# indiejoseph/speech-distill

Measured on AMD Instinct MI355X. Metric: distill-step tokens/sec (student seq_len=512), higher is better.
Workload: dtype bf16; 1 GPU; BASELINE config 2: Qwen3-0.6B-shape student + SoulX-1.7B-shape teacher (random init), V=159488, batch 4/GPU, seq_len 512, top_k 128, T=2.0 alpha=0.5, student fwd+bwd + teacher fwd + top-K + KL/CE; global_batch=4, seq_len=512, parallelism=single

## Files before the change

### include/sd_hip.h

```cpp
#pragma once
#include <stdint.h>
#ifdef __cplusplus
extern "C" {
#endif

#define SD_OK 0
#define SD_ERR_SHAPE (-1)
#define SD_ERR_ALIGN (-2)
#define SD_ERR_UNSUPPORTED (-3)
#define SD_ERR_NO_TEACHER (-4)
#define SD_ERR_WORKSPACE (-5)

#define SD_DTYPE_BF16 0
#define SD_DTYPE_F32 1

int sd_abi_version(void);

int sd_gemm_bf16(const void* A, const void* B, void* C, const void* R, int M, int N, int K, int64_t lda,
                 int64_t ldb, int64_t ldc, int64_t ldr, int trans_a, int trans_b, void* stream);

int sd_gemm_splitk_plan(int M, int N, int K);
int64_t sd_gemm_splitk_workspace_bytes(int M, int N, int K);
int sd_gemm_bf16_splitk(const void* A, const void* B, void* C, const void* R, int M, int N, int K, int64_t lda,
                        int64_t ldb, int64_t ldc, int64_t ldr, int trans_a, int trans_b, void* workspace,
// ... 60 lines not shown
int sd_qknorm_rope_bwd(const void* dqk, const void* qkv, const void* q_gain, const void* k_gain, const void* cos_tab,
                       const void* sin_tab, void* dqkv, void* dq_gain, void* dk_gain, int accumulate_dw, void* workspace,
                       int M, int T, int Hq, int Hkv, float eps, void* stream);

int sd_swiglu_fwd(const void* gate_up, void* act, int M, int I, void* stream);
int sd_swiglu_bwd(const void* dact, const void* gate_up, void* dgate_up, int M, int I, void* stream);

int sd_embedding_fwd(const int64_t* ids, const void* E, void* x, int M, int H, int V, void* stream);
int sd_embedding_bwd(const int64_t* ids, const void* dx, void* dE, int M, int H, int V, float scale, void* stream);
int sd_rows_scatter(const void* src, const int64_t* rows, void* dst, int n, int M, int H, void* stream);

int sd_attn_fwd(const void* q, const void* k, const void* v, void* o, float* lse, const int32_t* kv_len, int64_t ldq,
                int64_t ldk, int64_t ldv, int64_t ldo, int B, int T, int Hq, int Hkv, int head_dim, float scale,
                void* stream);
int sd_attn_bwd(const void* q, const void* k, const void* v, const void* o, const void* d_o, const float* lse,
                float* delta, void* dq, void* dk, void* dv, const int32_t* kv_len, int64_t ldq, int64_t ldk, int64_t ldv,
                int64_t ldo, int64_t lddq, int64_t lddk, int64_t lddv, int B, int T, int Hq, int Hkv, int head_dim,
                float scale, void* stream);

int sd_attn_bwd2(const void* q, const void* k, const void* v, const void* o, const void* d_o, const float* lse,
                 float* delta, void* dq, void* dk, void* dv, const int32_t* kv_len, int64_t ldq, int64_t ldk, int64_t ldv,
                 int64_t ldo, int64_t lddq, int64_t lddk, int64_t lddv, int B, int T, int Hq, int Hkv, int head_dim,
                 float scale, void* side_stream, void* stream);

int sd_logsoftmax_topk(const void* logits, void* top_v, void* top_i, float* lse_out, int rows, int64_t row_stride,
                       int V, int K, int dtype, void* stream);

int sd_loss_rows(const int64_t* labels, const int64_t* speech_mask, const int64_t* mask_a, const int64_t* mask_b,
                 int64_t* rows, int64_t* row_labels, int32_t* meta, int B, int T, void* stream);

int64_t sd_kdloss_stats_bytes(int B, int T);
int sd_kdloss_fwd(const void* student_logits, const void* teacher_logits, const void* top_k_v, const void* top_k_i,
                  const int64_t* labels, const uint8_t* speech_mask, void* row_stats, float* loss_out, int B, int T, int V,
                  int K, float temperature, float alpha, int dtype, void* stream);
int sd_kdloss_bwd(const void* student_logits, const void* teacher_logits, const void* top_k_v, const void* top_k_i,
                  const int64_t* labels, const void* row_stats, const float* loss_out, const float* grad_total,
                  void* grad_logits, int B, int T, int V, int K, float temperature, float alpha, int dtype, void* stream);

int sd_kdloss_fwd_rows(const void* student_logits, const void* teacher_logits, const void* top_k_v, const void* top_k_i,
                       const int64_t* row_labels, void* row_stats, float* loss_out, int R, int V, int K,
                       float temperature, float alpha, int dtype, void* stream);
int sd_kdloss_bwd_rows(const void* student_logits, const void* teacher_logits, const void* top_k_v, const void* top_k_i,
                       const int64_t* row_labels, const void* row_stats, const float* loss_out, const float* grad_total,
                       void* grad_logits, int R, int V, int K, float temperature, float alpha, int dtype, void* stream);

#define SD_SUMSQ_PARTIALS 2048
// ... 86 lines not shown
```

### speech_distill_amd/_lib.py

```python
from __future__ import annotations

import ctypes as C
import os

_HERE = os.path.dirname(os.path.abspath(__file__))
_LIB = None

ERRORS = {-1: "SD_ERR_SHAPE", -2: "SD_ERR_ALIGN", -3: "SD_ERR_UNSUPPORTED", -4: "SD_ERR_NO_TEACHER",
          -5: "SD_ERR_WORKSPACE"}


class SdHipError(RuntimeError):
    pass


def lib_path() -> str:
    return os.environ.get("SD_HIP_LIB") or os.path.join(_HERE, "libsd_hip.so")


class Dims(C.Structure):
    _fields_ = [("vocab", C.c_int32), ("hidden", C.c_int32), ("inter", C.c_int32), ("layers", C.c_int32),
                ("n_q", C.c_int32), ("n_kv", C.c_int32), ("head_dim", C.c_int32), ("tied", C.c_int32),
                ("eps", C.c_float), ("pad_", C.c_int32)]

# ... 52 lines not shown
    "sd_rmsnorm_bwd_workspace_bytes": (_i64, [_i, _i]),
    "sd_rmsnorm_bwd": (_i, [_vp, _vp, _vp, _vp, _vp, _vp, _vp, _i, _vp, _i, _i, _vp]),
    "sd_gemm_swiglu": (_i, [_vp, _vp, _vp, _vp, _i, _i, _i, _vp]),
    "sd_gemm_qkv_rope": (_i, [_vp, _vp, _vp, _vp, _vp, _vp, _vp, _vp, _i, _i, _i, _i, _i, _f, _vp]),
    "sd_embedding_fwd_ssq": (_i, [_vp, _vp, _vp, _vp, _i, _i, _i, _vp]),
    "sd_gemm_bf16_ssq": (_i, [_vp, _vp, _vp, _vp, _vp, _i, _i, _i, _i64, _i64, _i64, _i64, _vp]),
    "sd_gemm_qkv_rope_rs": (_i, [_vp, _vp, _vp, _vp, _vp, _vp, _vp, _vp, _vp, _i, _i, _i, _i, _i, _f, _vp]),
    "sd_gemm_swiglu_rs": (_i, [_vp, _vp, _vp, _vp, _vp, _f, _i, _i, _i, _vp]),
    "sd_qwen3_fold_supported": (_i, [C.POINTER(Dims)]),
    "sd_gemm_bf16_splitk_partial": (_i, [_vp, _vp, _vp, _i, _i, _i, _i64, _i64, _i64, _i, _i, _vp, _i64, _vp, _vp]),
    "sd_rmsnorm_bwd_slabs": (_i, [_vp, _i, _vp, _vp, _vp, _vp, _vp, _vp, _i, _vp, _i, _i, _vp, _vp, _vp]),
    "sd_rmsnorm_bwd2": (_i, [_vp, _vp, _vp, _vp, _vp, _vp, _vp, _i, _vp, _i, _i, _vp, _vp, _vp]),
    "sd_qknorm_rope_bwd2": (_i, [_vp, _vp, _vp, _vp, _vp, _vp, _vp, _vp, _vp, _i, _vp, _i, _i, _i, _i, _f, _vp, _vp, _vp]),
    "sd_qknorm_rope_fwd": (_i, [_vp, _vp, _vp, _vp, _vp, _vp, _i, _i, _i, _i, _f, _vp]),
    "sd_qknorm_rope_bwd_workspace_bytes": (_i64, [_i, _i, _i]),
    "sd_qknorm_rope_bwd": (_i, [_vp, _vp, _vp, _vp, _vp, _vp, _vp, _vp, _vp, _i, _vp, _i, _i, _i, _i, _f, _vp]),
    "sd_swiglu_fwd": (_i, [_vp, _vp, _i, _i, _vp]),
    "sd_swiglu_bwd": (_i, [_vp, _vp, _vp, _i, _i, _vp]),
    "sd_embedding_fwd": (_i, [_vp, _vp, _vp, _i, _i, _i, _vp]),
    "sd_embedding_bwd": (_i, [_vp, _vp, _vp, _i, _i, _i, _f, _vp]),
    "sd_attn_fwd": (_i, [_vp, _vp, _vp, _vp, _vp, _vp, _i64, _i64, _i64, _i64, _i, _i, _i, _i, _i, _f, _vp]),
    "sd_attn_bwd": (_i, [_vp] * 11 + [_i64] * 7 + [_i, _i, _i, _i, _i, _f, _vp]),
    "sd_attn_bwd2": (_i, [_vp] * 11 + [_i64] * 7 + [_i, _i, _i, _i, _i, _f, _vp, _vp]),
    "sd_logsoftmax_topk": (_i, [_vp, _vp, _vp, _vp, _i, _i64, _i, _i, _i, _vp]),
    "sd_kdloss_stats_bytes": (_i64, [_i, _i]),
    "sd_kdloss_fwd": (_i, [_vp, _vp, _vp, _vp, _vp, _vp, _vp, _vp, _i, _i, _i, _i, _f, _f, _i, _vp]),
    "sd_kdloss_bwd": (_i, [_vp, _vp, _vp, _vp, _vp, _vp, _vp, _vp, _vp, _i, _i, _i, _i, _f, _f, _i, _vp]),
    "sd_gemm_grouped_tn": (_i, [_vp, _i, _i, _i, _vp]),
    "sd_gemm_swiglu_bwd": (_i, [_vp, _vp, _vp, _vp, _i, _i, _i, _vp]),
    "sd_gemm_odx_delta": (_i, [_vp, _vp, _vp, _vp, _i64, _vp, _i, _i, _i, _i, _vp]),
    "sd_kdloss_fwd_rows": (_i, [_vp, _vp, _vp, _vp, _vp, _vp, _vp, _i, _i, _i, _f, _f, _i, _vp]),
    "sd_kdloss_bwd_rows": (_i, [_vp, _vp, _vp, _vp, _vp, _vp, _vp, _vp, _vp, _i, _i, _i, _f, _f, _i, _vp]),
    "sd_rows_scatter": (_i, [_vp, _vp, _vp, _i, _i, _i, _vp]),
    "sd_loss_rows": (_i, [_vp, _vp, _vp, _vp, _vp, _vp, _vp, _i, _i, _vp]),
    "sd_rmsnorm_bwd_partial_rows": (_i, [_i, _i]),
    "sd_qknorm_rope_bwd_partial_rows": (_i, [_i, _i, _i]),
    "sd_colsum_reduce_batch": (_i, [_vp, _i, _vp]),
    "sd_sumsq_bf16": (_i, [_vp, _i64, _vp, _vp, _vp]),
    "sd_adamw_bf16": (_i, [_vp, _vp, _vp, _vp, _i64, _f, _f, _f, _f, _f, _i, _vp, _f, _vp]),
    "sd_lora_plan_bytes": (_i64, [_i]),
    "sd_lora_plan_build": (_i, [C.POINTER(LoraTarget), _i, _i, _vp, _i64]),
    "sd_lora_merge": (_i, [_vp, _vp, _vp]),
    "sd_lora_project": (_i, [_vp, _vp, _vp]),
    "sd_adamw_f32_shadow": (_i, [_vp, _vp, _vp, _vp, _vp, _vp, _f, _i64, _f, _f, _f, _f, _f, _i, _vp, _f, _vp]),
    "sd_streams_overlap": (_i, [_vp, _vp, _f, C.POINTER(C.c_int)]),
    "sd_prof_begin": (_i, []),
# ... 68 lines not shown
```

### speech_distill_amd/csrc/sd_attn.hip

```cpp
#include <type_traits>
#include "sd_common.cuh"
#include "../../include/sd_hip.h"
#include "sd_prof.h"
#include "sd_debug.h"
#include "sd_events.h"

namespace {

constexpr int D = 128;
constexpr int TILE = 64 * D * 2;
constexpr float NEG = -1.0e30f;
constexpr float LOG2E = 1.4426950408889634f;

SD_DEV int f_swz(int row) { return ((row & 3) << 2) | ((row >> 2) & 3); }

template <int NP = 4>
struct TileDma {
  int voff[NP];
  long row_bytes;
#if defined(__HIP_DEVICE_COMPILE__)
  __amdgpu_buffer_rsrc_t rsrc;
#endif
  SD_DEV void init(const bf16* g, long ld, int rows, int w, int lane) {
    row_bytes = ld * 2;
// ... 33 lines not shown
  sd_u64 raw[8];
#pragma unroll
  for (int db = 0; db < 4; ++db) {
    const int ch = db * 4 + chl;
    lds_tr16_pair_asm(raw[2 * db], raw[2 * db + 1], aA + ((ch ^ sA) << 4), aB + ((ch ^ sB) << 4));
  }
  lds_tr_wait8(raw);
#pragma unroll
  for (int db = 0; db < 4; ++db) out[db] = cat8_u64(raw[2 * db], raw[2 * db + 1]);
}

SD_DEV void tr_issue4(const char* lds, int rb, int lane, sd_u64 (&raw)[8]) {
  const int gi = lane >> 4, i = lane & 15, q4 = i >> 2, pp = i & 3;
  const int rA = rb + 4 * (gi >> 1) + q4, rB = rA + 8;
  const int sA = f_swz(rA), sB = f_swz(rB);
  const unsigned base = lds_addr(lds) + 8 * (pp & 1);
  const unsigned aA = base + rA * 256, aB = base + rB * 256;
  const int chl = (gi & 1) * 2 + (pp >> 1);
#pragma unroll
  for (int db = 0; db < 4; ++db) {
    const int ch = db * 4 + chl;
    lds_tr16_pair_asm(raw[2 * db], raw[2 * db + 1], aA + ((ch ^ sA) << 4), aB + ((ch ^ sB) << 4));
  }
}
SD_DEV void tr_finish4(sd_u64 (&raw)[8], bf16x8 (&out)[4]) {
  lds_tr_wait8(raw);
#pragma unroll
  for (int db = 0; db < 4; ++db) out[db] = cat8_u64(raw[2 * db], raw[2 * db + 1]);
}

SD_DEV float halves_max(float x) {
  float a = x, b = x;
  asm volatile("s_nop 1\n\tv_permlane32_swap_b32 %0, %1\n\ts_nop 0" : "+v"(a), "+v"(b));
  return fmaxf(a, b);
}

SD_DEV bf16x8 acc_frag(const f32x16& p, int s) {
  bf16x8 r;
#pragma unroll
  for (int j = 0; j < 8; ++j) r[j] = (bf16)p[8 * s + j];
  return r;
}

SD_DEV int acc_row(int reg, int h) { return (reg & 3) + 8 * (reg >> 2) + 4 * h; }

SD_DEV void store_tile_rows(char* img, const f32x16 (&acc)[4], float mul, bf16* g_row0, long ld, int rows_valid, int lane) {
// ... 568 lines not shown
          for (int db = 0; db < 4; ++db) acc[db] = mfma32(kt4[db], df, acc[db]);
        }
      }
    }
  }
  asm volatile("s_waitcnt vmcnt(0)" ::: "memory");
  __syncthreads();
  float* xo = (float*)smem + (long)w * 64 * 64;
  if (half == 1) {
#pragma unroll
    for (int db = 0; db < 4; ++db)
#pragma unroll
      for (int e = 0; e < 16; ++e) xo[(db * 16 + e) * 64 + lane] = acc[db][e];
  }
  __syncthreads();
  if (half == 1 || !active) return;
#pragma unroll
  for (int db = 0; db < 4; ++db)
#pragma unroll
    for (int e = 0; e < 16; ++e) acc[db][e] += xo[(db * 16 + e) * 64 + lane];
  store_tile_rows((char*)xo, acc, scale, dQ + (tok0 + q0w) * lddq + hq * D, lddq, T - q0w, lane);
}

__global__ __launch_bounds__(512) void attn_bwd_dkv_kernel(const bf16* __restrict__ Q, const bf16* __restrict__ Kp,
                                                           const bf16* __restrict__ Vp, const bf16* __restrict__ dO,
                                                           const float* __restrict__ LSE, const float* __restrict__ delta,
                                                           bf16* __restrict__ dK, bf16* __restrict__ dV,
                                                           const int* __restrict__ kv_len, long ldq, long ldk, long ldv,
                                                           long ldo, long lddk, long lddv, int T, int Hq, int Hkv,
                                                           float scale) {
  __shared__ __attribute__((aligned(16))) char smem[8 * TILE + 1024];
  const int lane = lane_id(), w8 = wave_id_uniform();
  const int grp = w8 >> 2, sub = w8 & 1, rh = (w8 >> 1) & 1;
  const int sw = w8 & 3;
  const int G = Hq / Hkv;
  const int n64 = (T + 63) / 64;
  const AttnWg wg = attn_wg((int)blockIdx.x, (n64 + 1) / 2, 1, Hkv, (int)gridDim.x / (((n64 + 1) / 2) * Hkv));
  const int hkv = wg.hkv, b = wg.b;
  const int kbA = wg.pair, kbB = n64 - 1 - wg.pair;
  const bool active = grp == 0 || kbB != kbA;
  const int k0w = (grp == 0 ? kbA : kbB) * 64 + 32 * sub;
  const int r = lane & 31, h = lane >> 5;
  const int klen = kv_len ? max(1, min(kv_len[b], T)) : T;
  const long tok0 = (long)b * T;
  const int key = k0w + r;
  const bool key_ok = key < klen;
  const float c = scale * LOG2E;
  char* const ksm = smem;
  char* const vsm = smem + 2 * TILE;
  char* const ring = smem + 4 * TILE;
  float* const stat = (float*)(smem + 8 * TILE);
  {
    TileDma<> kvd;
    kvd.init((grp ? Vp + tok0 * ldv : Kp + tok0 * ldk) + hkv * D, grp ? ldv : ldk, T, sw, lane);
// ... 46 lines not shown
    const int qb0 = (qt0 + it % per_head) * 64 + 32 * rh;
    if (!active || qb0 + 31 < k0w) continue;
    f32x16 s, dp;
#pragma unroll
    for (int e = 0; e < 16; ++e) { s[e] = 0.f; dp[e] = 0.f; }
#pragma unroll
    for (int st = 0; st < 8; ++st) {
      s = mfma32(row_frag(qs, 32 * rh, st, lane), row_frag(ksm, 64 * grp + 32 * sub, st, lane), s);
      dp = mfma32(row_frag(dos, 32 * rh, st, lane), row_frag(vsm, 64 * grp + 32 * sub, st, lane), dp);
    }
#pragma unroll
    for (int g4 = 0; g4 < 4; ++g4) {
      const f32x4 l2 = *(const f32x4*)&stat[buf * 128 + 32 * rh + 8 * g4 + 4 * h];
      const f32x4 dl = *(const f32x4*)&stat[buf * 128 + 64 + 32 * rh + 8 * g4 + 4 * h];
#pragma unroll
      for (int e = 0; e < 4; ++e) {
        const int qq = qb0 + 8 * g4 + 4 * h + e;
        const bool vis = key_ok && key <= qq && qq < T;
        const float p = vis ? __builtin_amdgcn_exp2f(s[4 * g4 + e] * c - l2[e]) : 0.f;
        s[4 * g4 + e] = p;
        dp[4 * g4 + e] = p * (dp[4 * g4 + e] - dl[e]);
      }
    }
#pragma unroll
    for (int ss = 0; ss < 2; ++ss) {
      bf16x8 t4[4];
      const bf16x8 pf = acc_frag(s, ss);
      tr_frag4(dos, 32 * rh + 16 * ss, lane, t4);
#pragma unroll
      for (int db = 0; db < 4; ++db) dv[db] = mfma32(t4[db], pf, dv[db]);
      const bf16x8 df = acc_frag(dp, ss);
      tr_frag4(qs, 32 * rh + 16 * ss, lane, t4);
#pragma unroll
      for (int db = 0; db < 4; ++db) dk[db] = mfma32(t4[db], df, dk[db]);
    }
  }
  asm volatile("s_waitcnt vmcnt(0) lgkmcnt(0)" ::: "memory");
  __syncthreads();
  float* xo = (float*)smem + (long)(grp * 2 + sub) * 64 * 64;
#pragma unroll
  for (int round = 0; round < 2; ++round) {
    f32x16* acc = round ? dv : dk;
    if (rh == 1) {
#pragma unroll
      for (int db = 0; db < 4; ++db)
#pragma unroll
        for (int e = 0; e < 16; ++e) xo[(db * 16 + e) * 64 + lane] = acc[db][e];
    }
    __syncthreads();
    if (rh == 0) {
#pragma unroll
      for (int db = 0; db < 4; ++db)
#pragma unroll
        for (int e = 0; e < 16; ++e) acc[db][e] += xo[(db * 16 + e) * 64 + lane];
    }
    __syncthreads();
  }
  if (rh == 0 && active) {
    store_tile_rows((char*)xo, dk, scale, dK + (tok0 + k0w) * lddk + hkv * D, lddk, T - k0w, lane);
    store_tile_rows((char*)xo + 8192, dv, 1.f, dV + (tok0 + k0w) * lddv + hkv * D, lddv, T - k0w, lane);
  }
}

int check_common(int B, int T, int Hq, int Hkv, long ldq, long ldk, long ldv, long ldo) {
  if (B <= 0 || T <= 0 || Hq <= 0 || Hkv <= 0 || (Hq % Hkv)) return SD_ERR_SHAPE;
  if ((ldq | ldk | ldv | ldo) & 7) return SD_ERR_ALIGN;
  return 0;
}

}

#ifdef SD_STAMPS
static unsigned long long* g_attn_stamps = nullptr;
extern "C" void sd_debug_attn_stamp_buffer(void* p) { g_attn_stamps = (unsigned long long*)p; }
#define SD_ATT_STAMP_ARG , g_attn_stamps
#else
#define SD_ATT_STAMP_ARG
#endif


extern "C" int sd_attn_fwd(const void* q, const void* k, const void* v, void* o, float* lse, const int32_t* kv_len,
                           int64_t ldq, int64_t ldk, int64_t ldv, int64_t ldo, int B, int T, int Hq, int Hkv,
                           int head_dim, float scale, void* stream) {
  if (head_dim != D) return SD_ERR_UNSUPPORTED;
  if (int e = check_common(B, T, Hq, Hkv, ldq, ldk, ldv, ldo)) return e;
  if (((uintptr_t)q | (uintptr_t)k | (uintptr_t)v | (uintptr_t)o) & 15) return SD_ERR_ALIGN;
  SdProfScope prof(SD_K_ATTN_FWD, 2.0 * B * Hq * (double)T * T * D, (hipStream_t)stream);
  const dim3 grid((((T + 63) / 64 + 1) / 2) * Hq * B);
  const bool pipe = (g_sd_debug.attn_variant & 2) || (!(g_sd_debug.attn_variant & 1) && T >= 1024);
  if (pipe) {
    hipLaunchKernelGGL(attn_fwd_pipe_kernel, grid, dim3(512), 0, (hipStream_t)stream, (const bf16*)q, (const bf16*)k,
                       (const bf16*)v, (bf16*)o, lse, kv_len, ldq, ldk, ldv, ldo, T, Hq, Hkv, scale SD_ATT_STAMP_ARG);
    SD_CHECK_LAUNCH();
    return 0;
  }
  hipLaunchKernelGGL(attn_fwd_kernel, grid, dim3(512), 0, (hipStream_t)stream, (const bf16*)q,
                     (const bf16*)k, (const bf16*)v, (bf16*)o, lse, kv_len, ldq, ldk, ldv, ldo, T, Hq, Hkv, scale SD_ATT_STAMP_ARG);
  SD_CHECK_LAUNCH();
  return 0;
}

extern "C" int sd_attn_bwd2(const void* q, const void* k, const void* v, const void* o, const void* d_o, const float* lse,
                            float* delta, void* dq, void* dk, void* dv, const int32_t* kv_len, int64_t ldq, int64_t ldk,
                            int64_t ldv, int64_t ldo, int64_t lddq, int64_t lddk, int64_t lddv, int B, int T, int Hq,
                            int Hkv, int head_dim, float scale, void* side_stream, void* stream) {
  if (head_dim != D) return SD_ERR_UNSUPPORTED;
  if (int e = check_common(B, T, Hq, Hkv, ldq, ldk, ldv, ldo)) return e;
  if ((lddq | lddk | lddv) & 7) return SD_ERR_ALIGN;
  hipStream_t st = (hipStream_t)stream, s2 = (hipStream_t)side_stream;
  SdEventLease lease;
  if (s2 && !(lease.set = sd_lease_events())) return SD_ERR_WORKSPACE;
  hipEvent_t* g_attn_ev = lease.set ? lease.set->ev : nullptr;
  const long total = (long)B * T * Hq;
  if (o) {
    hipLaunchKernelGGL(attn_delta_kernel, dim3((unsigned)((total + 15) / 16)), dim3(256), 0, st, (const bf16*)d_o,
                       (const bf16*)o, delta, ldo, T, Hq, total);
    SD_CHECK_LAUNCH();
  }
  hipStream_t sq = s2 ? s2 : st;
  if (s2) {
    if (hipEventRecord(g_attn_ev[0], st) != hipSuccess || hipStreamWaitEvent(s2, g_attn_ev[0], 0) != hipSuccess)
      return SD_ERR_WORKSPACE;
  }
  {
    SdProfScope prof2(SD_K_ATTN_BWD_DQ, 3.0 * B * Hq * (double)T * T * D, sq);
    hipLaunchKernelGGL(attn_bwd_dq_kernel, dim3((((T + 63) / 64 + 1) / 2) * Hq * B), dim3(512), 0, sq, (const bf16*)q, (const bf16*)k,
                       (const bf16*)v, (const bf16*)d_o, lse, (const float*)delta, (bf16*)dq, kv_len, ldq, ldk, ldv, ldo,
                       lddq, T, Hq, Hkv, scale);
  }
  SD_CHECK_LAUNCH();
  {
    SdProfScope prof(SD_K_ATTN_BWD_DKV, 4.0 * B * Hq * (double)T * T * D, st);
    hipLaunchKernelGGL(attn_bwd_dkv_kernel, dim3((((T + 63) / 64 + 1) / 2) * Hkv * B), dim3(512), 0, st, (const bf16*)q,
                       (const bf16*)k, (const bf16*)v, (const bf16*)d_o, lse, (const float*)delta, (bf16*)dk, (bf16*)dv,
                       kv_len, ldq, ldk, ldv, ldo, lddk, lddv, T, Hq, Hkv, scale);
  }
  SD_CHECK_LAUNCH();
  if (s2) {
    if (hipEventRecord(g_attn_ev[1], s2) != hipSuccess || hipStreamWaitEvent(st, g_attn_ev[1], 0) != hipSuccess)
      return SD_ERR_WORKSPACE;
  }
  return 0;
}

extern "C" int sd_attn_bwd(const void* q, const void* k, const void* v, const void* o, const void* d_o, const float* lse,
                           float* delta, void* dq, void* dk, void* dv, const int32_t* kv_len, int64_t ldq, int64_t ldk,
                           int64_t ldv, int64_t ldo, int64_t lddq, int64_t lddk, int64_t lddv, int B, int T, int Hq,
                           int Hkv, int head_dim, float scale, void* stream) {
  return sd_attn_bwd2(q, k, v, o, d_o, lse, delta, dq, dk, dv, kv_len, ldq, ldk, ldv, ldo, lddq, lddk, lddv, B, T, Hq,
                      Hkv, head_dim, scale, nullptr, stream);
}
```

### speech_distill_amd/csrc/sd_debug.h

```cpp
#pragma once

struct SdDebug {
  int gemm_force_bm = 0, gemm_force_nst = 0;
  int gemm_checked_staging = 0;
  int gemm_p256_unpaired = 0;
  int gemm_cu_budget = 0;
  int gemm_no_persist = 0, gemm_no_p256 = 0;
  int gemm_p256_min_tiles = 1024;
  int gemm_group_m = 0;
  int gemm_tn_stag_min = 1024;
  int gemm_splitk_min_kt = 96, gemm_splitk_min_slice = 24;
  int gemm_splitk_max = 0;
  int gemm_fwd_cu_budget = 0;
  int gemm_persist_balance = 0;
  int gemm_no_table = 0;
  int gemm_fwd_bump = 0;
  int model_fuse_student_swiglu = 0;
  int model_shared_layers = -1, model_shared_layers_train = -1;
  int model_overlap_mask = 31;
  int topk_nt = 0;
  int qk_bwd_blocks = 512;
  int attn_variant = 0;
};
extern SdDebug g_sd_debug;

extern thread_local int t_sd_shared_gpu;
struct SdSharedGpuScope {
  int prev;
  explicit SdSharedGpuScope(int on) : prev(t_sd_shared_gpu) { t_sd_shared_gpu = on; }
  ~SdSharedGpuScope() { t_sd_shared_gpu = prev; }
};
```

### speech_distill_amd/csrc/sd_debug.hip

```cpp
#include <stdint.h>
#include <string.h>
#include "../../include/sd_hip.h"
#include "../../include/sd_hip_debug.h"
#include "sd_debug.h"

SdDebug g_sd_debug;
thread_local int t_sd_shared_gpu = 0;

namespace {
struct Key { const char* name; int SdDebug::*field; };
const Key kKeys[] = {
    {"gemm.force_bm", &SdDebug::gemm_force_bm},
    {"gemm.force_nst", &SdDebug::gemm_force_nst},
    {"gemm.checked_staging", &SdDebug::gemm_checked_staging},
    {"gemm.p256_unpaired", &SdDebug::gemm_p256_unpaired},
    {"gemm.cu_budget", &SdDebug::gemm_cu_budget},
    {"gemm.no_persist", &SdDebug::gemm_no_persist},
    {"gemm.no_p256", &SdDebug::gemm_no_p256},
    {"gemm.p256_min_tiles", &SdDebug::gemm_p256_min_tiles},
    {"gemm.group_m", &SdDebug::gemm_group_m},
    {"gemm.tn_stag_min", &SdDebug::gemm_tn_stag_min},
    {"gemm.splitk_min_kt", &SdDebug::gemm_splitk_min_kt},
    {"gemm.splitk_min_slice", &SdDebug::gemm_splitk_min_slice},
    {"gemm.splitk_max", &SdDebug::gemm_splitk_max},
    {"gemm.no_table", &SdDebug::gemm_no_table},
    {"gemm.persist_balance", &SdDebug::gemm_persist_balance},
    {"gemm.fwd_cu_budget", &SdDebug::gemm_fwd_cu_budget},
    {"gemm.fwd_bump", &SdDebug::gemm_fwd_bump},
    {"model.fuse_student_swiglu", &SdDebug::model_fuse_student_swiglu},
    {"model.overlap_mask", &SdDebug::model_overlap_mask},
    {"model.shared_layers", &SdDebug::model_shared_layers},
    {"model.shared_layers_train", &SdDebug::model_shared_layers_train},
    {"topk.nt", &SdDebug::topk_nt},
    {"qk_bwd.blocks", &SdDebug::qk_bwd_blocks},
    {"attn.variant", &SdDebug::attn_variant},
};
}

extern "C" int sd_debug_set(const char* key, int64_t value) {
  if (!key) return SD_ERR_SHAPE;
  if (!strcmp(key, "reset")) { g_sd_debug = SdDebug{}; return SD_OK; }
  for (const Key& k : kKeys)
    if (!strcmp(key, k.name)) {
      if (k.field == &SdDebug::gemm_splitk_min_slice && value < 1) value = 1;
      g_sd_debug.*(k.field) = (int)value;
      return SD_OK;
    }
  return SD_ERR_UNSUPPORTED;
}

extern "C" int64_t sd_debug_get(const char* key) {
  if (key)
    for (const Key& k : kKeys)
      if (!strcmp(key, k.name)) return g_sd_debug.*(k.field);
  return INT64_MIN;
}

extern "C" int sd_debug_keys(char* buf, int cap) {
// ... 10 lines not shown
```

### speech_distill_amd/csrc/sd_model.hip

```cpp
#include <hip/hip_runtime.h>
#include <stdint.h>
#include <stdlib.h>
#include "../../include/sd_hip.h"
#include "sd_events.h"
#include "sd_debug.h"

namespace {

inline int64_t al(int64_t x) { return (x + 255) & ~(int64_t)255; }

struct Sizes {
  int M, h, I, QD, KD, QKV, QK, V, L, Hq, Hkv;
  int64_t x, rstd, qkv, qk, ao, lse, gu, act;
  Sizes(const sd_qwen3_dims* d, int B, int T) {
    M = B * T; h = d->hidden; I = d->inter; Hq = d->n_q; Hkv = d->n_kv;
    QD = Hq * d->head_dim; KD = Hkv * d->head_dim; QKV = QD + 2 * KD; QK = QD + KD; V = d->vocab; L = d->layers;
    x = al((int64_t)M * h * 2); rstd = al((int64_t)M * 4); qkv = al((int64_t)M * QKV * 2); qk = al((int64_t)M * QK * 2);
    ao = al((int64_t)M * QD * 2); lse = al((int64_t)B * Hq * T * 4); gu = al((int64_t)M * 2 * I * 2);
    act = al((int64_t)M * I * 2);
  }
  int64_t per_layer() const { return 4 * x + 2 * rstd + qkv + qk + ao + lse + gu + act; }
  int64_t tail() const { return 3 * x + rstd; }
  int64_t ssq() const { return al((int64_t)M * 16 * 4); }
  int64_t body(int save) const {
    return save == SD_SAVE_ALL ? (int64_t)L * per_layer() : save == SD_SAVE_LAYER_INPUTS ? (int64_t)L * x + 2 * per_layer()
                                                                                          : per_layer() + x;
  }
};

struct LayerActs {
  char *x_in, *rstd1, *xn1, *qkv, *qk, *ao, *lse, *x_mid, *rstd2, *xn2, *gu, *act;
};

LayerActs carve(const Sizes& s, char* p) {
  LayerActs a;
  a.x_in = p; p += s.x;
  a.rstd1 = p; p += s.rstd;
  a.xn1 = p; p += s.x;
  a.qkv = p; p += s.qkv;
  a.qk = p; p += s.qk;
  a.ao = p; p += s.ao;
  a.lse = p; p += s.lse;
  a.x_mid = p; p += s.x;
  a.rstd2 = p; p += s.rstd;
  a.xn2 = p; p += s.x;
  a.gu = p; p += s.gu;
  a.act = p; p += s.act;
  return a;
}

struct BwdScratch {
  char *dxa[2], *dxb[2], *dqkv[2], *dgu[2], *ws_norm2[2], *ws_qk[2], *ws_norm1[2];
  char *dxn, *dqk, *dao, *delta, *dact, *ws_norm, *ws_splitk;
  int64_t total, splitk_bytes;
  BwdScratch(const Sizes& s, char* p) {
    char* p0 = p;
    for (int i = 0; i < 2; ++i) {
      dxa[i] = p; p += s.x;
      dxb[i] = p; p += s.x;
      dqkv[i] = p; p += s.qkv;
      dgu[i] = p; p += s.gu;
      ws_norm2[i] = p; p += al(sd_rmsnorm_bwd_workspace_bytes(s.M, s.h));
      ws_qk[i] = p; p += al(sd_qknorm_rope_bwd_workspace_bytes(s.M, s.Hq, s.Hkv));
      ws_norm1[i] = p; p += al(sd_rmsnorm_bwd_workspace_bytes(s.M, s.h));
    }
    dxn = p; p += s.x;
    dqk = p; p += s.qk;
    dao = p; p += s.ao;
    delta = p; p += s.lse;
    dact = p; p += s.act;
    ws_norm = p; p += al(sd_rmsnorm_bwd_workspace_bytes(s.M, s.h));
    splitk_bytes = sd_gemm_splitk_workspace_bytes(s.M, s.h, s.V);
    for (int k : {s.QKV, 2 * s.I, s.QD, s.I}) {
      const int64_t b1 = sd_gemm_splitk_workspace_bytes(s.M, s.h, k);
      splitk_bytes = b1 > splitk_bytes ? b1 : splitk_bytes;
    }
    ws_splitk = p; p += al(splitk_bytes);
    total = p - p0;
  }
};

#define RUN(call) do { int e__ = (call); if (e__) return e__; } while (0)

LayerActs layer_acts(const Sizes& s, char* base, int l, int save) {
  if (save == SD_SAVE_ALL) return carve(s, base + (int64_t)l * s.per_layer());
  LayerActs a = carve(s, base + (int64_t)s.L * s.x + (int64_t)(l & 1) * s.per_layer());
  a.x_in = base + (int64_t)l * s.x;
  return a;
}

int layer_forward(const sd_qwen3_dims* d, const Sizes& s, const LayerActs& a, const sd_qwen3_layer& w, char* x_out,
                  bool keep_gu, const int32_t* kv_len, const void* cos_tab, const void* sin_tab, int B, int T,
                  void* stream) {
  const float scale = 0.08838834764831845f;
  RUN(sd_rmsnorm_fwd(a.x_in, w.ln1, a.xn1, (float*)a.rstd1, s.M, s.h, d->eps, stream));
  int rc = sd_gemm_qkv_rope(a.xn1, w.wqkv, a.qkv, a.qk, w.q_gain, w.k_gain, cos_tab, sin_tab, s.M, T, s.Hq, s.Hkv, s.h,
                            d->eps, stream);
  if (rc == SD_ERR_UNSUPPORTED) {
    RUN(sd_gemm_bf16(a.xn1, w.wqkv, a.qkv, nullptr, s.M, s.QKV, s.h, s.h, s.h, s.QKV, 0, 0, 0, stream));
    RUN(sd_qknorm_rope_fwd(a.qkv, w.q_gain, w.k_gain, cos_tab, sin_tab, a.qk, s.M, T, s.Hq, s.Hkv, d->eps, stream));
// ... 241 lines not shown
      const int rc = sd_gemm_swiglu_bwd(dx_in, w.wdown, a.gu, dgu, s.M, s.I, s.h, stream);
      if (rc == SD_ERR_UNSUPPORTED) {
        RUN(sd_gemm_bf16(dx_in, w.wdown, b.dact, nullptr, s.M, s.I, s.h, s.h, s.I, s.I, 0, 0, 1, stream));
        RUN(sd_swiglu_bwd(b.dact, a.gu, dgu, s.M, s.I, stream));
      } else if (rc) {
        return rc;
      }
    }
    if (!grouped) SIGNAL(1);
    RUN(sd_gemm_bf16_splitk_partial(dgu, w.wgu, b.dxn, s.M, s.h, 2 * s.I, 2 * s.I, s.h, s.h, 0, 1, b.ws_splitk,
                                    b.splitk_bytes, &nsp, stream));
    if (!grouped) RUN(sd_gemm_bf16(dgu, a.xn2, gw.wgu, ACC(gw.wgu), 2 * s.I, s.h, s.M, 2 * s.I, s.h, s.h, s.h, 1, 1, wstream));
    NORM_BWD(a.x_mid, w.ln2, (const float*)a.rstd2, dx_in, dxb, batch_gains ? nullptr : gw.ln2, b.ws_norm2[P],
             (ovl & 2) ? side_stream : nullptr, s2 ? (void*)g_ev[8] : nullptr);
    if (!grouped) SIGNAL(2);
    const void* o_for_delta = a.ao;
    {
      const int rc = sd_gemm_odx_delta(dxb, w.wo, b.dao, a.ao, s.QD, (float*)b.delta, s.M, T, s.Hq, s.h, stream);
      if (rc == SD_ERR_UNSUPPORTED) RUN(sd_gemm_bf16(dxb, w.wo, b.dao, nullptr, s.M, s.QD, s.h, s.h, s.QD, s.QD, 0, 0, 1, stream));
      else if (rc) return rc;
      else o_for_delta = nullptr;
    }
    if (!grouped) RUN(sd_gemm_bf16(dxb, a.ao, gw.wo, ACC(gw.wo), s.h, s.QD, s.M, s.h, s.QD, s.QD, s.QD, 1, 1, wstream));
    RUN(sd_attn_bwd2(a.qk, a.qk + (int64_t)s.QD * 2, a.qkv + (int64_t)(s.QD + s.KD) * 2, o_for_delta, b.dao, (const float*)a.lse,
                    (float*)b.delta, b.dqk, b.dqk + (int64_t)s.QD * 2, dqkv + (int64_t)(s.QD + s.KD) * 2, kv_len, s.QK,
                    s.QK, s.QKV, s.QD, s.QK, s.QK, s.QKV, B, T, s.Hq, s.Hkv, 128, scale, (ovl & 4) ? side_stream : nullptr, stream));
    RUN(sd_qknorm_rope_bwd2(b.dqk, a.qkv, w.q_gain, w.k_gain, cos_tab, sin_tab, dqkv, batch_gains ? nullptr : gw.q_gain,
                            batch_gains ? nullptr : gw.k_gain, acc, b.ws_qk[P], s.M, T, s.Hq, s.Hkv, d->eps,
                            (ovl & 2) ? side_stream : nullptr, s2 ? (void*)g_ev[9] : nullptr, stream));
    SIGNAL(3);
    if (grouped) {
      sd_gemm_problem pr[4] = {
          {dqkv, a.xn1, gw.wqkv, s.QKV, s.h, s.h, s.QKV, s.h},
          {dgu, a.xn2, gw.wgu, 2 * s.I, s.h, s.h, 2 * s.I, s.h},
          {dx_in, a.act, gw.wdown, s.h, s.I, s.I, s.h, s.I},
          {dxb, a.ao, gw.wo, s.h, s.QD, s.QD, s.h, s.QD}};
      const int rc = sd_gemm_grouped_tn(pr, 4, s.M, acc, wstream);
      if (rc == SD_ERR_UNSUPPORTED) {
        for (const sd_gemm_problem& q : pr)
          RUN(sd_gemm_bf16(q.A, q.B, q.C, acc ? q.C : nullptr, q.M, q.N, s.M, q.lda, q.ldb, q.ldc, q.ldc, 1, 1, wstream));
      } else if (rc) {
        return rc;
      }
      if (!batch_gains && s2 && hipEventRecord(g_ev[10 + P], s2) != hipSuccess) return SD_ERR_WORKSPACE;
    } else {
      RUN(sd_gemm_bf16(dqkv, a.xn1, gw.wqkv, ACC(gw.wqkv), s.QKV, s.h, s.M, s.QKV, s.h, s.h, s.h, 1, 1, wstream));
    }
    RUN(sd_gemm_bf16_splitk_partial(dqkv, w.wqkv, b.dxn, s.M, s.h, s.QKV, s.QKV, s.h, s.h, 0, 1, b.ws_splitk,
                                    b.splitk_bytes, &nsp, stream));
// ... 39 lines not shown
```

### speech_distill_amd/ops.py

```python
from __future__ import annotations

import ctypes as C
import os

import torch

from ._lib import check, load_lib

BF16, F32 = 0, 1


def _stream():
    return torch.cuda.current_stream().cuda_stream


def _p(t):
    return 0 if t is None else t.data_ptr()


_SIDE_STREAMS = {}
_ROLES_ACTIVE_TOGETHER = {"teacher": (), "dw": ("comm",), "comm": ("dw",), "h2d": ("teacher",)}


def streams_overlap(a, b, spin_us=200.0):
# ... 149 lines not shown
    V, H = dE.shape
    check(load_lib().sd_embedding_bwd(ids.data_ptr(), dx.data_ptr(), dE.data_ptr(), ids.numel(), H, V, float(scale),
                                      _stream()),
          "sd_embedding_bwd")
    return dE


def attn_fwd(q, k, v, B, T, Hq, Hkv, kv_len=None):
    M = B * T
    o = torch.empty(M, Hq * 128, dtype=torch.bfloat16, device=q.device)
    lse = torch.empty(B, Hq, T, dtype=torch.float32, device=q.device)
    check(load_lib().sd_attn_fwd(q.data_ptr(), k.data_ptr(), v.data_ptr(), o.data_ptr(), lse.data_ptr(), _p(kv_len),
                                 q.stride(0), k.stride(0), v.stride(0), o.stride(0), B, T, Hq, Hkv, 128, 128 ** -0.5,
                                 _stream()), "sd_attn_fwd")
    return o, lse


def attn_bwd(q, k, v, o, do, lse, B, T, Hq, Hkv, kv_len=None, delta=None):
    if o is None and delta is None:
        raise ValueError("attn_bwd: either o or a precomputed delta")
    if delta is None:
        delta = torch.empty_like(lse)
    dq, dk, dv = torch.zeros_like(q), torch.zeros_like(k), torch.zeros_like(v)
    check(load_lib().sd_attn_bwd(q.data_ptr(), k.data_ptr(), v.data_ptr(), _p(o), do.data_ptr(), lse.data_ptr(),
                                 delta.data_ptr(), dq.data_ptr(), dk.data_ptr(), dv.data_ptr(), _p(kv_len), q.stride(0),
                                 k.stride(0), v.stride(0), do.stride(0), dq.stride(0), dk.stride(0), dv.stride(0), B, T, Hq,
                                 Hkv, 128, 128 ** -0.5, _stream()), "sd_attn_bwd")
    return dq, dk, dv


def logsoftmax_topk(logits, k, vocab_size=None):
    _need(logits, None, "logits")
    lead = logits.shape[:-1]
    Vt = logits.shape[-1]
    V = Vt if vocab_size is None else min(int(vocab_size), Vt)
    if (Vt % 8) or (logits.data_ptr() % 16):
        logits = logits[..., :V].contiguous()
        Vt = V
    rows = logits.numel() // Vt
    tv = torch.empty(*lead, k, dtype=torch.float16, device=logits.device)
    ti = torch.empty(*lead, k, dtype=torch.int32, device=logits.device)
    check(load_lib().sd_logsoftmax_topk(logits.data_ptr(), tv.data_ptr(), ti.data_ptr(), 0, rows, Vt, V, k, _dt(logits),
                                        _stream()), "sd_logsoftmax_topk")
    return tv, ti


class KDLossFn(torch.autograd.Function):

    @staticmethod
    def forward(ctx, student_logits, labels, teacher_logits, top_v, top_i, speech_mask, temperature, alpha, inplace_grad):
# ... 323 lines not shown
```

Before: 104,400 tokens/s.

## Materialize dS in dK/dV attention backward and compute dQ as a GEMM

For short sequences (T<=512, the default), the dK/dV backward kernel now writes the bf16 dS tiles for each query head into a workspace laid out in triangular pairs. A new dQ kernel then computes dQ = dS·K as a plain GEMM. Previously a separate dQ kernel recomputed QK^T, the softmax and dP. This removes roughly two thirds of the dQ FLOPs at the cost of extra global-memory traffic for dS. It also drops the side-stream overlap between the dQ and dK/dV kernels, since the two now run sequentially.

```diff
diff --git a/include/sd_hip.h b/include/sd_hip.h
--- a/include/sd_hip.h
+++ b/include/sd_hip.h
@@ -106,6 +106,11 @@
                  float* delta, void* dq, void* dk, void* dv, const int32_t* kv_len, int64_t ldq, int64_t ldk, int64_t ldv,
                  int64_t ldo, int64_t lddq, int64_t lddk, int64_t lddv, int B, int T, int Hq, int Hkv, int head_dim,
                  float scale, void* side_stream, void* stream);
+int sd_attn_bwd3(const void* q, const void* k, const void* v, const void* o, const void* d_o, const float* lse,
+                 float* delta, void* dq, void* dk, void* dv, const int32_t* kv_len, int64_t ldq, int64_t ldk, int64_t ldv,
+                 int64_t ldo, int64_t lddq, int64_t lddk, int64_t lddv, int B, int T, int Hq, int Hkv, int head_dim,
+                 float scale, void* ws, int64_t ws_bytes, void* side_stream, void* stream);
+int64_t sd_attn_bwd_workspace_bytes(int B, int T, int Hq);
 
 int sd_logsoftmax_topk(const void* logits, void* top_v, void* top_i, float* lse_out, int rows, int64_t row_stride,
                        int V, int K, int dtype, void* stream);
diff --git a/speech_distill_amd/_lib.py b/speech_distill_amd/_lib.py
--- a/speech_distill_amd/_lib.py
+++ b/speech_distill_amd/_lib.py
@@ -98,6 +98,8 @@
     "sd_attn_fwd": (_i, [_vp, _vp, _vp, _vp, _vp, _vp, _i64, _i64, _i64, _i64, _i, _i, _i, _i, _i, _f, _vp]),
     "sd_attn_bwd": (_i, [_vp] * 11 + [_i64] * 7 + [_i, _i, _i, _i, _i, _f, _vp]),
     "sd_attn_bwd2": (_i, [_vp] * 11 + [_i64] * 7 + [_i, _i, _i, _i, _i, _f, _vp, _vp]),
+    "sd_attn_bwd3": (_i, [_vp] * 11 + [_i64] * 7 + [_i, _i, _i, _i, _i, _f, _vp, _i64, _vp, _vp]),
+    "sd_attn_bwd_workspace_bytes": (_i64, [_i, _i, _i]),
     "sd_logsoftmax_topk": (_i, [_vp, _vp, _vp, _vp, _i, _i64, _i, _i, _i, _vp]),
     "sd_kdloss_stats_bytes": (_i64, [_i, _i]),
     "sd_kdloss_fwd": (_i, [_vp, _vp, _vp, _vp, _vp, _vp, _vp, _vp, _i, _i, _i, _i, _f, _f, _i, _vp]),
diff --git a/speech_distill_amd/csrc/sd_attn.hip b/speech_distill_amd/csrc/sd_attn.hip
--- a/speech_distill_amd/csrc/sd_attn.hip
+++ b/speech_distill_amd/csrc/sd_attn.hip
@@ -79,6 +79,13 @@
     const int ch = db * 4 + chl;
     lds_tr16_pair_asm(raw[2 * db], raw[2 * db + 1], aA + ((ch ^ sA) << 4), aB + ((ch ^ sB) << 4));
   }
+}
+SD_DEV void tr_issue1(const char* lds, int rb, int db, int lane, sd_u64 (&raw)[2]) {
+  const int gi = lane >> 4, i = lane & 15, q4 = i >> 2, pp = i & 3;
+  const int rA = rb + 4 * (gi >> 1) + q4, rB = rA + 8;
+  const unsigned base = lds_addr(lds) + 8 * (pp & 1);
+  const int ch = db * 4 + (gi & 1) * 2 + (pp >> 1);
+  lds_tr16_pair_asm(raw[0], raw[1], base + rA * 256 + ((ch ^ f_swz(rA)) << 4), base + rB * 256 + ((ch ^ f_swz(rB)) << 4));
 }
 SD_DEV void tr_finish4(sd_u64 (&raw)[8], bf16x8 (&out)[4]) {
   lds_tr_wait8(raw);
@@ -693,14 +700,20 @@
   store_tile_rows((char*)xo, acc, scale, dQ + (tok0 + q0w) * lddq + hq * D, lddq, T - q0w, lane);
 }
 
+__host__ __device__ inline long ds_pair_offset(int p, int n64) { return (long)p * n64 - (long)p * (p - 1) / 2; }
+__host__ __device__ inline long ds_tile_index(int b, int hq, int p, int kt, int n64, int Hq) {
+  return ((long)b * Hq + hq) * ds_pair_offset((n64 + 1) / 2, n64) + ds_pair_offset(p, n64) + kt;
+}
+
+template <bool WRITE_DS>
 __global__ __launch_bounds__(512) void attn_bwd_dkv_kernel(const bf16* __restrict__ Q, const bf16* __restrict__ Kp,
                                                            const bf16* __restrict__ Vp, const bf16* __restrict__ dO,
                                                            const float* __restrict__ LSE, const float* __restrict__ delta,
                                                            bf16* __restrict__ dK, bf16* __restrict__ dV,
                                                            const int* __restrict__ kv_len, long ldq, long ldk, long ldv,
                                                            long ldo, long lddk, long lddv, int T, int Hq, int Hkv,
-                                                           float scale) {
-  __shared__ __attribute__((aligned(16))) char smem[8 * TILE + 1024];
+                                                           float scale, bf16* __restrict__ dS) {
+  __shared__ __attribute__((aligned(16))) char smem[8 * TILE + 1024 + (WRITE_DS ? 8 * 2048 : 0)];
   const int lane = lane_id(), w8 = wave_id_uniform();
   const int grp = w8 >> 2, sub = w8 & 1, rh = (w8 >> 1) & 1;
   const int sw = w8 & 3;
@@ -793,6 +806,31 @@
         dp[4 * g4 + e] = p * (dp[4 * g4 + e] - dl[e]);
       }
     }
+    if constexpr (WRITE_DS) {
+      {
+        char* xr = smem + 8 * TILE + 1024 + w8 * 2048 + r * 64 + 8 * h;
+        const int sx = (r >> 2) & 3;
+#pragma unroll
+        for (int ss = 0; ss < 2; ++ss) {
+          const bf16x8 df = acc_frag(dp, ss);
+          *(bf16x4*)(xr + (((2 * ss) ^ sx) << 4)) = bf16x4{df[0], df[1], df[2], df[3]};
+          *(bf16x4*)(xr + (((2 * ss + 1) ^ sx) << 4)) = bf16x4{df[4], df[5], df[6], df[7]};
+        }
+      }
+      const int qt = qt0 + it % per_head, hq = hkv * G + it / per_head;
+      const int pr = min(qt, n64 - 1 - qt);
+      const int col = (qt == n64 - 1 - pr ? 0 : 64) + 32 * rh;
+      bf16* gt = dS + ds_tile_index(b, hq, pr, k0w >> 6, n64, Hq) * (64 * D) + (long)(k0w & 63) * D + col;
+      asm volatile("s_waitcnt lgkmcnt(0)" ::: "memory");
+      const char* xs = smem + 8 * TILE + 1024 + w8 * 2048;
+      const int c = lane & 3;
+#pragma unroll
+      for (int i = 0; i < 2; ++i) {
+        const int row = 16 * i + (lane >> 2);
+        const bf16x8 v = *(const bf16x8*)(xs + row * 64 + ((c ^ ((row >> 2) & 3)) << 4));
+        *(bf16x8*)(gt + (long)row * D + 8 * c) = v;
+      }
+    }
 #pragma unroll
     for (int ss = 0; ss < 2; ++ss) {
       bf16x8 t4[4];
@@ -831,6 +869,87 @@
     store_tile_rows((char*)xo, dk, scale, dK + (tok0 + k0w) * lddk + hkv * D, lddk, T - k0w, lane);
     store_tile_rows((char*)xo + 8192, dv, 1.f, dV + (tok0 + k0w) * lddv + hkv * D, lddv, T - k0w, lane);
   }
+}
+
+__global__ __launch_bounds__(512) void attn_bwd_dq_gemm_kernel(const bf16* __restrict__ Kp, const bf16* __restrict__ dS,
+                                                               bf16* __restrict__ dQ, long ldk, long lddq, int T, int Hq,
+                                                               int Hkv, float scale) {
+  __shared__ __attribute__((aligned(16))) char smem[8 * TILE];
+  const int lane = lane_id(), w8 = wave_id_uniform();
+  const int grp = w8 >> 2, rb = w8 & 1, half = (w8 >> 1) & 1;
+  const int w = grp * 2 + rb;
+  const int n64 = (T + 63) / 64, npairs = (n64 + 1) / 2;
+  const AttnWg wg = attn_wg((int)blockIdx.x, npairs, Hq / Hkv, Hkv, (int)gridDim.x / (npairs * Hq));
+  const int tA = n64 - 1 - wg.pair, tB = wg.pair;
+  const bool active = grp == 0 || tB != tA;
+  const int hkv = wg.hkv, b = wg.b;
+  const int hq = hkv * (Hq / Hkv) + wg.member_head;
+  const int q0w = (grp == 0 ? tA : tB) * 64 + 32 * rb;
+  const long tok0 = (long)b * T;
+  f32x16 acc[4];
+#pragma unroll
+  for (int db = 0; db < 4; ++db)
+#pragma unroll
+    for (int e = 0; e < 16; ++e) acc[db][e] = 0.f;
+
+  const int kv_hi = min(tA * 64 + 64, T);
+  const int nkv = (kv_hi + 63) / 64;
+  const int nit = (nkv + 1) >> 1;
+  TileDma<> kd, sd;
+  kd.init(Kp + tok0 * ldk + hkv * D, ldk, T, w, lane);
+  sd.init(dS + ds_tile_index(b, hq, wg.pair, 0, n64, Hq) * (64 * D), D, nkv * 64, w, lane);
+  char* ring = smem + half * 4 * TILE;
+  kd.issue(half * 64, ring, w);
+  sd.issue(half * 64, ring + TILE, w);
+  int cur_i = 0;
+  for (int i = 0; i < nit; ++i) {
+    asm volatile("s_waitcnt vmcnt(0)" ::: "memory");
+    __builtin_amdgcn_s_barrier();
+    asm volatile("" ::: "memory");
+    if ((2 * (i + 1) + half) * 64 < kv_hi) {
+      char* nx = ring + (cur_i ^ 1) * 2 * TILE;
+      kd.issue((2 * (i + 1) + half) * 64, nx, w);
+      sd.issue((2 * (i + 1) + half) * 64, nx + TILE, w);
+    }
+    const char* ks = ring + cur_i * 2 * TILE;
+    const char* dss = ks + TILE;
+    cur_i ^= 1;
+    const int kv0 = (2 * i + half) * 64;
+    if (active && kv0 < kv_hi) {
+#pragma unroll
+      for (int kb2 = 0; kb2 < 2; ++kb2) {
+        if (kv0 + 32 * kb2 > q0w + 31) continue;
+#pragma unroll
+        for (int ss = 0; ss < 2; ++ss) {
+          bf16x8 kt4[4];
+          sd_u64 rk[8], rd[2];
+          tr_issue4(ks, kb2 * 32 + 16 * ss, lane, rk);
+          tr_issue1(dss, kb2 * 32 + 16 * ss, grp * 2 + rb, lane, rd);
+          asm volatile("s_waitcnt lgkmcnt(0)" : "+v"(rd[0]), "+v"(rd[1]));
+          tr_finish4(rk, kt4);
+          const bf16x8 df = cat8_u64(rd[0], rd[1]);
+#pragma unroll
+          for (int db = 0; db < 4; ++db) acc[db] = mfma32(kt4[db], df, acc[db]);
+        }
+      }
+    }
+  }
+  asm volatile("s_waitcnt vmcnt(0)" ::: "memory");
+  __syncthreads();
+  float* xo = (float*)smem + (long)w * 64 * 64;
+  if (half == 1) {
+#pragma unroll
+    for (int db = 0; db < 4; ++db)
+#pragma unroll
+      for (int e = 0; e < 16; ++e) xo[(db * 16 + e) * 64 + lane] = acc[db][e];
+  }
+  __syncthreads();
+  if (half == 1 || !active) return;
+#pragma unroll
+  for (int db = 0; db < 4; ++db)
+#pragma unroll
+    for (int e = 0; e < 16; ++e) acc[db][e] += xo[(db * 16 + e) * 64 + lane];
+  store_tile_rows((char*)xo, acc, scale, dQ + (tok0 + q0w) * lddq + hq * D, lddq, T - q0w, lane);
 }
 
 int check_common(int B, int T, int Hq, int Hkv, long ldq, long ldk, long ldv, long ldo) {
@@ -871,23 +990,53 @@
   return 0;
 }
 
-extern "C" int sd_attn_bwd2(const void* q, const void* k, const void* v, const void* o, const void* d_o, const float* lse,
-                            float* delta, void* dq, void* dk, void* dv, const int32_t* kv_len, int64_t ldq, int64_t ldk,
-                            int64_t ldv, int64_t ldo, int64_t lddq, int64_t lddk, int64_t lddv, int B, int T, int Hq,
-                            int Hkv, int head_dim, float scale, void* side_stream, void* stream) {
+constexpr int kDsMaxT = 512;
+
+static bool attn_bwd_uses_ds(int T) {
+  return g_sd_debug.attn_bwd_ds == 2 || (g_sd_debug.attn_bwd_ds == 0 && T <= kDsMaxT);
+}
+
+extern "C" int64_t sd_attn_bwd_workspace_bytes(int B, int T, int Hq) {
+  if (B <= 0 || T <= 0 || Hq <= 0 || !attn_bwd_uses_ds(T)) return 0;
+  const int n64 = (T + 63) / 64;
+  return (int64_t)B * Hq * ds_pair_offset((n64 + 1) / 2, n64) * TILE;
+}
+
+static int attn_bwd_impl(const void* q, const void* k, const void* v, const void* o, const void* d_o, const float* lse,
+                         float* delta, void* dq, void* dk, void* dv, const int32_t* kv_len, int64_t ldq, int64_t ldk,
+                         int64_t ldv, int64_t ldo, int64_t lddq, int64_t lddk, int64_t lddv, int B, int T, int Hq,
+                         int Hkv, int head_dim, float scale, void* ds_ws, void* side_stream, void* stream) {
   if (head_dim != D) return SD_ERR_UNSUPPORTED;
   if (int e = check_common(B, T, Hq, Hkv, ldq, ldk, ldv, ldo)) return e;
   if ((lddq | lddk | lddv) & 7) return SD_ERR_ALIGN;
-  hipStream_t st = (hipStream_t)stream, s2 = (hipStream_t)side_stream;
-  SdEventLease lease;
-  if (s2 && !(lease.set = sd_lease_events())) return SD_ERR_WORKSPACE;
-  hipEvent_t* g_attn_ev = lease.set ? lease.set->ev : nullptr;
+  hipStream_t st = (hipStream_t)stream;
   const long total = (long)B * T * Hq;
   if (o) {
     hipLaunchKernelGGL(attn_delta_kernel, dim3((unsigned)((total + 15) / 16)), dim3(256), 0, st, (const bf16*)d_o,
                        (const bf16*)o, delta, ldo, T, Hq, total);
     SD_CHECK_LAUNCH();
   }
+  const int npairs = ((T + 63) / 64 + 1) / 2;
+  if (ds_ws) {
+    {
+      SdProfScope prof(SD_K_ATTN_BWD_DKV, 4.0 * B * Hq * (double)T * T * D, st);
+      hipLaunchKernelGGL(attn_bwd_dkv_kernel<true>, dim3(npairs * Hkv * B), dim3(512), 0, st, (const bf16*)q,
+                         (const bf16*)k, (const bf16*)v, (const bf16*)d_o, lse, (const float*)delta, (bf16*)dk, (bf16*)dv,
+                         kv_len, ldq, ldk, ldv, ldo, lddk, lddv, T, Hq, Hkv, scale, (bf16*)ds_ws);
+    }
+    SD_CHECK_LAUNCH();
+    {
+      SdProfScope prof2(SD_K_ATTN_BWD_DQ, 1.0 * B * Hq * (double)T * T * D, st);
+      hipLaunchKernelGGL(attn_bwd_dq_gemm_kernel, dim3(npairs * Hq * B), dim3(512), 0, st, (const bf16*)k,
+                         (const bf16*)ds_ws, (bf16*)dq, ldk, lddq, T, Hq, Hkv, scale);
+    }
+    SD_CHECK_LAUNCH();
+    return 0;
+  }
+  hipStream_t s2 = (hipStream_t)side_stream;
+  SdEventLease lease;
+  if (s2 && !(lease.set = sd_lease_events())) return SD_ERR_WORKSPACE;
+  hipEvent_t* g_attn_ev = lease.set ? lease.set->ev : nullptr;
   hipStream_t sq = s2 ? s2 : st;
   if (s2) {
     if (hipEventRecord(g_attn_ev[0], st) != hipSuccess || hipStreamWaitEvent(s2, g_attn_ev[0], 0) != hipSuccess)
@@ -895,16 +1044,16 @@
   }
   {
     SdProfScope prof2(SD_K_ATTN_BWD_DQ, 3.0 * B * Hq * (double)T * T * D, sq);
-    hipLaunchKernelGGL(attn_bwd_dq_kernel, dim3((((T + 63) / 64 + 1) / 2) * Hq * B), dim3(512), 0, sq, (const bf16*)q, (const bf16*)k,
+    hipLaunchKernelGGL(attn_bwd_dq_kernel, dim3(npairs * Hq * B), dim3(512), 0, sq, (const bf16*)q, (const bf16*)k,
                        (const bf16*)v, (const bf16*)d_o, lse, (const float*)delta, (bf16*)dq, kv_len, ldq, ldk, ldv, ldo,
                        lddq, T, Hq, Hkv, scale);
   }
   SD_CHECK_LAUNCH();
   {
     SdProfScope prof(SD_K_ATTN_BWD_DKV, 4.0 * B * Hq * (double)T * T * D, st);
-    hipLaunchKernelGGL(attn_bwd_dkv_kernel, dim3((((T + 63) / 64 + 1) / 2) * Hkv * B), dim3(512), 0, st, (const bf16*)q,
+    hipLaunchKernelGGL(attn_bwd_dkv_kernel<false>, dim3(npairs * Hkv * B), dim3(512), 0, st, (const bf16*)q,
                        (const bf16*)k, (const bf16*)v, (const bf16*)d_o, lse, (const float*)delta, (bf16*)dk, (bf16*)dv,
-                       kv_len, ldq, ldk, ldv, ldo, lddk, lddv, T, Hq, Hkv, scale);
+                       kv_len, ldq, ldk, ldv, ldo, lddk, lddv, T, Hq, Hkv, scale, (bf16*)nullptr);
   }
   SD_CHECK_LAUNCH();
   if (s2) {
@@ -912,6 +1061,29 @@
       return SD_ERR_WORKSPACE;
   }
   return 0;
+}
+
+extern "C" int sd_attn_bwd2(const void* q, const void* k, const void* v, const void* o, const void* d_o, const float* lse,
+                            float* delta, void* dq, void* dk, void* dv, const int32_t* kv_len, int64_t ldq, int64_t ldk,
+                            int64_t ldv, int64_t ldo, int64_t lddq, int64_t lddk, int64_t lddv, int B, int T, int Hq,
+                            int Hkv, int head_dim, float scale, void* side_stream, void* stream) {
+  return attn_bwd_impl(q, k, v, o, d_o, lse, delta, dq, dk, dv, kv_len, ldq, ldk, ldv, ldo, lddq, lddk, lddv, B, T, Hq,
+                       Hkv, head_dim, scale, nullptr, side_stream, stream);
+}
+
+extern "C" int sd_attn_bwd3(const void* q, const void* k, const void* v, const void* o, const void* d_o, const float* lse,
+                            float* delta, void* dq, void* dk, void* dv, const int32_t* kv_len, int64_t ldq, int64_t ldk,
+                            int64_t ldv, int64_t ldo, int64_t lddq, int64_t lddk, int64_t lddv, int B, int T, int Hq,
+                            int Hkv, int head_dim, float scale, void* ws, int64_t ws_bytes, void* side_stream,
+                            void* stream) {
+  void* ds_ws = nullptr;
+  if (attn_bwd_uses_ds(T)) {
+    const int64_t need = sd_attn_bwd_workspace_bytes(B, T, Hq);
+    if (!ws || ws_bytes < need || ((uintptr_t)ws & 15)) return SD_ERR_WORKSPACE;
+    ds_ws = ws;
+  }
+  return attn_bwd_impl(q, k, v, o, d_o, lse, delta, dq, dk, dv, kv_len, ldq, ldk, ldv, ldo, lddq, lddk, lddv, B, T, Hq,
+                       Hkv, head_dim, scale, ds_ws, side_stream, stream);
 }
 
 extern "C" int sd_attn_bwd(const void* q, const void* k, const void* v, const void* o, const void* d_o, const float* lse,
diff --git a/speech_distill_amd/csrc/sd_debug.h b/speech_distill_amd/csrc/sd_debug.h
--- a/speech_distill_amd/csrc/sd_debug.h
+++ b/speech_distill_amd/csrc/sd_debug.h
@@ -21,6 +21,7 @@
   int topk_nt = 0;
   int qk_bwd_blocks = 512;
   int attn_variant = 0;
+  int attn_bwd_ds = 0;
 };
 extern SdDebug g_sd_debug;
 
diff --git a/speech_distill_amd/csrc/sd_debug.hip b/speech_distill_amd/csrc/sd_debug.hip
--- a/speech_distill_amd/csrc/sd_debug.hip
+++ b/speech_distill_amd/csrc/sd_debug.hip
@@ -34,6 +34,7 @@
     {"topk.nt", &SdDebug::topk_nt},
     {"qk_bwd.blocks", &SdDebug::qk_bwd_blocks},
     {"attn.variant", &SdDebug::attn_variant},
+    {"attn.bwd_ds", &SdDebug::attn_bwd_ds},
 };
 }
 
diff --git a/speech_distill_amd/csrc/sd_model.hip b/speech_distill_amd/csrc/sd_model.hip
--- a/speech_distill_amd/csrc/sd_model.hip
+++ b/speech_distill_amd/csrc/sd_model.hip
@@ -10,9 +10,9 @@
 inline int64_t al(int64_t x) { return (x + 255) & ~(int64_t)255; }
 
 struct Sizes {
-  int M, h, I, QD, KD, QKV, QK, V, L, Hq, Hkv;
+  int M, h, I, QD, KD, QKV, QK, V, L, Hq, Hkv, B, T;
   int64_t x, rstd, qkv, qk, ao, lse, gu, act;
-  Sizes(const sd_qwen3_dims* d, int B, int T) {
+  Sizes(const sd_qwen3_dims* d, int B_, int T_) : B(B_), T(T_) {
     M = B * T; h = d->hidden; I = d->inter; Hq = d->n_q; Hkv = d->n_kv;
     QD = Hq * d->head_dim; KD = Hkv * d->head_dim; QKV = QD + 2 * KD; QK = QD + KD; V = d->vocab; L = d->layers;
     x = al((int64_t)M * h * 2); rstd = al((int64_t)M * 4); qkv = al((int64_t)M * QKV * 2); qk = al((int64_t)M * QK * 2);
@@ -51,8 +51,8 @@
 
 struct BwdScratch {
   char *dxa[2], *dxb[2], *dqkv[2], *dgu[2], *ws_norm2[2], *ws_qk[2], *ws_norm1[2];
-  char *dxn, *dqk, *dao, *delta, *dact, *ws_norm, *ws_splitk;
-  int64_t total, splitk_bytes;
+  char *dxn, *dqk, *dao, *delta, *dact, *ws_norm, *ws_splitk, *ws_ds;
+  int64_t total, splitk_bytes, ds_bytes;
   BwdScratch(const Sizes& s, char* p) {
     char* p0 = p;
     for (int i = 0; i < 2; ++i) {
@@ -76,6 +76,8 @@
       splitk_bytes = b1 > splitk_bytes ? b1 : splitk_bytes;
     }
     ws_splitk = p; p += al(splitk_bytes);
+    ds_bytes = sd_attn_bwd_workspace_bytes(s.B, s.T, s.Hq);
+    ws_ds = p; p += al(ds_bytes);
     total = p - p0;
   }
 };
@@ -363,9 +365,10 @@
       else o_for_delta = nullptr;
     }
     if (!grouped) RUN(sd_gemm_bf16(dxb, a.ao, gw.wo, ACC(gw.wo), s.h, s.QD, s.M, s.h, s.QD, s.QD, s.QD, 1, 1, wstream));
-    RUN(sd_attn_bwd2(a.qk, a.qk + (int64_t)s.QD * 2, a.qkv + (int64_t)(s.QD + s.KD) * 2, o_for_delta, b.dao, (const float*)a.lse,
+    RUN(sd_attn_bwd3(a.qk, a.qk + (int64_t)s.QD * 2, a.qkv + (int64_t)(s.QD + s.KD) * 2, o_for_delta, b.dao, (const float*)a.lse,
                     (float*)b.delta, b.dqk, b.dqk + (int64_t)s.QD * 2, dqkv + (int64_t)(s.QD + s.KD) * 2, kv_len, s.QK,
-                    s.QK, s.QKV, s.QD, s.QK, s.QK, s.QKV, B, T, s.Hq, s.Hkv, 128, scale, (ovl & 4) ? side_stream : nullptr, stream));
+                    s.QK, s.QKV, s.QD, s.QK, s.QK, s.QKV, B, T, s.Hq, s.Hkv, 128, scale, b.ws_ds, b.ds_bytes,
+                    (ovl & 4) ? side_stream : nullptr, stream));
     RUN(sd_qknorm_rope_bwd2(b.dqk, a.qkv, w.q_gain, w.k_gain, cos_tab, sin_tab, dqkv, batch_gains ? nullptr : gw.q_gain,
                             batch_gains ? nullptr : gw.k_gain, acc, b.ws_qk[P], s.M, T, s.Hq, s.Hkv, d->eps,
                             (ovl & 2) ? side_stream : nullptr, s2 ? (void*)g_ev[9] : nullptr, stream));
diff --git a/speech_distill_amd/ops.py b/speech_distill_amd/ops.py
--- a/speech_distill_amd/ops.py
+++ b/speech_distill_amd/ops.py
@@ -195,10 +195,13 @@
     if delta is None:
         delta = torch.empty_like(lse)
     dq, dk, dv = torch.zeros_like(q), torch.zeros_like(k), torch.zeros_like(v)
-    check(load_lib().sd_attn_bwd(q.data_ptr(), k.data_ptr(), v.data_ptr(), _p(o), do.data_ptr(), lse.data_ptr(),
-                                 delta.data_ptr(), dq.data_ptr(), dk.data_ptr(), dv.data_ptr(), _p(kv_len), q.stride(0),
-                                 k.stride(0), v.stride(0), do.stride(0), dq.stride(0), dk.stride(0), dv.stride(0), B, T, Hq,
-                                 Hkv, 128, 128 ** -0.5, _stream()), "sd_attn_bwd")
+    lib = load_lib()
+    nws = lib.sd_attn_bwd_workspace_bytes(B, T, Hq)
+    ws = torch.empty(nws, dtype=torch.uint8, device=q.device) if nws > 0 else None
+    check(lib.sd_attn_bwd3(q.data_ptr(), k.data_ptr(), v.data_ptr(), _p(o), do.data_ptr(), lse.data_ptr(),
+                           delta.data_ptr(), dq.data_ptr(), dk.data_ptr(), dv.data_ptr(), _p(kv_len), q.stride(0),
+                           k.stride(0), v.stride(0), do.stride(0), dq.stride(0), dk.stride(0), dv.stride(0), B, T, Hq,
+                           Hkv, 128, 128 ** -0.5, _p(ws), nws, None, _stream()), "sd_attn_bwd3")
     return dq, dk, dv
 
 
```

Result: no change. 104,100 tokens/s, median of 6 (-0.3%).
